# steineggerlab/unicore

Hardware: AMD Instinct MI355X
Metric: 3Di alignments/sec (cluster path) (higher is better)
Workload: dtype u16

## Files before the change

### unicore_amd/csrc/uc_prefilter.hip

```cpp
#include <hip/hip_runtime.h>

#include <algorithm>
#include <cstdlib>
#include <cstring>
#include <type_traits>

#include <rocprim/rocprim.hpp>

#include "uc_engine.h"

namespace uc {

constexpr uint32_t KMER_INVALID = 0xFFFFFFFFu;

struct KmerCfg {
    int koff[K];
    int span;
    int thr;
};

__device__ __forceinline__ uint32_t find_seq(const uint32_t *off, uint32_t lo, uint32_t hi, uint32_t p) {
    while (hi - lo > 1) {
        const uint32_t mid = lo + ((hi - lo) >> 1);
        if (off[mid] <= p) lo = mid; else hi = mid;
// ... 502 lines not shown
            if (base + k < key_cap) keys[base + k] = key;
        }
        __syncthreads();
    }
}

constexpr int FB_LOG2 = 19;
constexpr int FT = 1024;
constexpr int KPT = 4;
constexpr int FILTER_RPT = 2;
constexpr size_t filter_lds(int rpt) { return 2 * ((size_t)1 << FB_LOG2) / 8 + ((size_t)rpt * FT + 1) * 4 + (size_t)rpt * FT * 8 + 16 * 4 + 64; }

__global__ void __launch_bounds__(256) run_range_kernel(const DeviceDb db, uint32_t qbegin, uint32_t nq, uint32_t p0, const uint32_t *rpidx,
                                                        uint64_t n_runs, uint64_t *qr) {
    for (uint32_t i = blockIdx.x * 256 + threadIdx.x; i <= nq; i += gridDim.x * 256) {
        const uint32_t want = db.off[qbegin + i] - p0;
        uint64_t lo = 0, hi = n_runs;
        while (lo < hi) { const uint64_t m = (lo + hi) >> 1; if (rpidx[m] < want) lo = m + 1; else hi = m; }
        qr[i] = lo;
    }
}

__global__ void __launch_bounds__(256) run_order_key_kernel(uint32_t nq, const uint64_t *qr, uint32_t *key, uint32_t *idx) {
    for (uint32_t i = blockIdx.x * 256 + threadIdx.x; i < nq; i += gridDim.x * 256) {
        const uint64_t c = qr[i + 1] - qr[i];
        key[i] = 0xFFFFFFFFu - (uint32_t)min<uint64_t>(c, 0xFFFFFFFFull);
        idx[i] = i;
    }
}

template <bool C> struct TdType { using type = uint64_t; };
template <> struct TdType<true> { using type = uint32_t; };

template <bool C>
__global__ void __launch_bounds__(FT) filter_kernel(const DeviceDb db, uint32_t qbegin, uint32_t p0, const uint32_t *rpidx,
                                                    const uint64_t *rval, const uint64_t *qr, const uint32_t *order, const void *ent, KeyFmt fmt,
                                                    unsigned long long *region_cursor, void *region_v, uint64_t region_cap,
                                                    uint64_t *qbase, uint32_t *qsurv) {
    using TD = typename TdType<C>::type;
    struct __attribute__((aligned(4))) TD4 { TD v[KPT]; };
    TD *region = (TD *)region_v;
    extern __shared__ __attribute__((aligned(16))) uint32_t f_lds[];
    constexpr int BW = 1 << (FB_LOG2 - 5);
    constexpr int RPT = FILTER_RPT;
    constexpr int TR = RPT * FT;
    uint32_t *B1 = f_lds, *B2 = f_lds + BW;
    uint2 *s_run = (uint2 *)(f_lds + 2 * BW);
    uint32_t *s_pref = (uint32_t *)(s_run + TR);
    uint32_t *s_wsum = s_pref + TR + 1;
    uint64_t *s_misc = (uint64_t *)(((uintptr_t)(s_wsum + 16) + 7) & ~(uintptr_t)7);
    const int tid = threadIdx.x, lane = tid & 63, wv = tid >> 6;
    const uint32_t qi = order[blockIdx.x];
    const uint32_t q = qbegin + qi;
    const uint32_t plo = db.off[q] - p0;
    const uint64_t r0 = qr[qi], r1 = qr[qi + 1];
    TD *surv = region + region_cap;
    for (int w = tid; w < 2 * BW; w += FT) f_lds[w] = 0;
    if (r0 == r1) {
        if (tid == 0) { qbase[qi] = 0; qsurv[qi] = 0; }
        return;
    }

    uint64_t pf_rv[RPT] = {};
    uint32_t pf_pi[RPT] = {};
    auto prefetch_tile = [&](uint64_t tile) {
#pragma unroll
        for (int j = 0; j < RPT; j++) {
            const uint64_t r = tile + (uint64_t)RPT * tid + j;
            if (r < r1) { pf_rv[j] = rval[r]; pf_pi[j] = rpidx[r]; }
        }
    };
    auto load_tile = [&](uint64_t tile) {
        uint32_t c[RPT], csum = 0;
#pragma unroll
        for (int j = 0; j < RPT; j++) {
            const uint64_t r = tile + (uint64_t)RPT * tid + j;
            c[j] = r < r1 ? (uint32_t)(pf_rv[j] >> 32) : 0u;
            csum += c[j];
        }
        uint32_t inc = csum;
        for (int o = 1; o < 64; o <<= 1) {
            const uint32_t up = (uint32_t)__shfl_up((int)inc, o, 64);
            if (lane >= o) inc += up;
        }
        if (lane == 63) s_wsum[wv] = inc;
        __syncthreads();
        uint32_t woff = 0;
        for (int w = 0; w < wv; w++) woff += s_wsum[w];
        uint32_t pre = woff + inc - csum;
#pragma unroll
        for (int j = 0; j < RPT; j++) {
            s_pref[RPT * tid + j] = pre;
// ... 160 lines not shown
    __syncthreads();
    auto slot2_of = [&](uint64_t key, uint32_t &h2) -> uint32_t {
        const uint32_t x = (uint32_t)key * 0xC2B2AE35u ^ (uint32_t)(key >> 32) * 0x27D4EB2Fu;
        h2 = ((x ^ (x >> 13)) * 0x165667B1u) >> (32 - FB_LOG2);
        return (x * 0x9E3779B1u) >> (32 - FB_LOG2);
    };
    for (uint32_t k = tid; k < n1; k += FT) {
        uint32_t g;
        const uint32_t h = slot2_of(surv[base + k], g), bit = 1u << (h & 31), gbit = 1u << (g & 31);
        const uint32_t old = atomicOr(&B1[h >> 5], bit);
        if (old & bit) atomicOr(&B2[h >> 5], bit);
        const uint32_t gold = atomicOr(&B1[g >> 5], gbit);
        if (gold & gbit) atomicOr(&B2[g >> 5], gbit);
    }
    __syncthreads();
    const uint32_t n1r = (n1 + 63) / 64 * 64;
    for (uint32_t k = tid; k < n1r; k += FT) {
        TD key = 0;
        bool keep = false;
        if (k < n1) {
            key = surv[base + k];
            uint32_t g;
            const uint32_t h = slot2_of(key, g);
            keep = ((B2[h >> 5] >> (h & 31)) & (B2[g >> 5] >> (g & 31))) & 1u;
        }
        const uint64_t m = __builtin_amdgcn_ballot_w64(keep);
        if (m) {
            uint32_t s0 = 0;
            if (lane == 0) s0 = atomicAdd(cur2, (uint32_t)__popcll(m));
            s0 = (uint32_t)__shfl((int)s0, 0, 64);
            if (keep) region[base + s0 + (uint32_t)__popcll(m & ((1ull << lane) - 1ull))] = key;
        }
    }
    __syncthreads();
    if (tid == 0) { qbase[qi] = base; qsurv[qi] = *cur2; }
}

template <bool C>
__global__ void __launch_bounds__(256) compact_kernel(const void *region_v, const uint64_t *qbase, const uint32_t *qsurv,
                                                      const uint64_t *soff, uint32_t nq, KeyFmt fmt, uint64_t *out) {
    using TD = typename TdType<C>::type;
    const TD *region = (const TD *)region_v;
    const uint64_t dmask = (1ull << fmt.dbits) - 1;
    for (uint32_t b = blockIdx.x; b < nq; b += gridDim.x) {
        const uint64_t src = qbase[b], dst = soff[b];
        const uint32_t n = qsurv[b];
        const uint64_t qbits = (uint64_t)b << (fmt.tbits + fmt.dbits);
        for (uint32_t k = threadIdx.x; k < n; k += 256) {
            const uint64_t td = region[src + k];
            out[dst + k] = C ? (qbits | (((td >> fmt.dbits) + fmt.tbase) << fmt.dbits) | (td & dmask)) : (qbits | td);
        }
    }
}

__global__ void __launch_bounds__(256) diag_select_kernel(const uint64_t *keys, uint64_t n, int min_hits, KeyFmt fmt, uint32_t qbegin,
                                                          unsigned long long *n_cand, uint64_t cap,
                                                          uint32_t *cq, uint32_t *ct, int32_t *cd, uint32_t mirror_q0, uint8_t *wflag) {
    constexpr int DS_SLOTS = 128, DS_DRAIN = 64;
    __shared__ uint32_t s_q[4][DS_SLOTS], s_t[4][DS_SLOTS];
    __shared__ int32_t s_d[4][DS_SLOTS];
    const int lane = threadIdx.x & 63, wv = threadIdx.x >> 6;
    const uint64_t dmask = (1ull << fmt.dbits) - 1, tmask = (1ull << fmt.tbits) - 1;
    const uint64_t nround = (n + 255) / 256 * 256;
    uint32_t staged = 0;
    auto drain = [&]() {
        uint32_t blo = 0, bhi = 0;
        if (lane == 0) {
            const unsigned long long b = atomicAdd(n_cand, (unsigned long long)staged);
// ... 11 lines not shown
    };
    __shared__ uint64_t s_v1[4][64], s_v2[4][64];
    for (uint64_t i = (uint64_t)blockIdx.x * 256 + threadIdx.x; i < nround; i += (uint64_t)gridDim.x * 256) {
        bool cand = false, deferred = false;
        int best_d = 0, last_d = 0;
        uint64_t grp = 0;
        const uint64_t wbase = i - (uint64_t)lane;
        const bool valid = i < n;
        const uint64_t k = valid ? keys[i] : ~0ull;
        uint64_t kp = (uint64_t)__shfl_up((unsigned long long)k, 1, 64);
        if (lane == 0) kp = (valid && i > 0) ? keys[i - 1] : ~k;
        const bool run_start = valid && kp != k;
        const bool grp_start = valid && (i == 0 || (kp >> fmt.dbits) != (k >> fmt.dbits));
        const uint64_t starts = __builtin_amdgcn_ballot_w64(run_start), gstarts = __builtin_amdgcn_ballot_w64(grp_start);
        const uint64_t above = lane == 63 ? 0ull : (~0ull << (lane + 1));
        const uint64_t wend = wbase + 64 < n ? wbase + 64 : n;
        if (grp_start && !(gstarts & above) && wend < n) {
            const uint64_t far = wend + 63 < n ? wend + 63 : n - 1;
            deferred = (keys[far] >> fmt.dbits) == (k >> fmt.dbits);
        }
        const bool long_tail = __builtin_amdgcn_ballot_w64(deferred) != 0;
        uint64_t v1 = 0, v2 = 0;
        if (run_start) {
            const uint64_t nx = starts & above;
            uint64_t cnt;
            if (nx) cnt = (uint64_t)(__builtin_ctzll(nx) - lane);
            else {
                uint64_t e = wend;
                const uint64_t lim = wend + 64 < n ? wend + 64 : n;
                if (!long_tail) while (e < lim && keys[e] == k) e++;
                cnt = e - i;
            }
            const uint64_t d = k & dmask;
            v1 = (cnt << 32) | (0xFFFFFFFFull - d);
            v2 = (cnt << 32) | d;
        }
        s_v1[wv][lane] = v1; s_v2[wv][lane] = v2;
        __builtin_amdgcn_wave_barrier();
        if (grp_start) {
            grp = k >> fmt.dbits;
            const uint64_t ng = gstarts & above;
            const int gend = ng ? __builtin_ctzll(ng) : 64;
            uint64_t b1 = 0, b2 = 0;
            uint64_t runs = starts & (~0ull << lane) & (gend == 64 ? ~0ull : ((1ull << gend) - 1ull));
            while (runs) {
                const int r = __builtin_ctzll(runs);
                runs &= runs - 1;
                const uint64_t a = s_v1[wv][r], c2 = s_v2[wv][r];
                b1 = a > b1 ? a : b1; b2 = c2 > b2 ? c2 : b2;
            }
            if (gend == 64 && wend < n && !deferred) {
                uint64_t e = wend;
                const uint64_t kw = keys[wend - 1];
                while (e < n && keys[e] == kw) e++;
                while (e < n && (keys[e] >> fmt.dbits) == grp) {
                    const uint64_t kb = keys[e];
                    uint64_t f = e + 1;
                    while (f < n && keys[f] == kb) f++;
                    const uint64_t cnt = f - e, d = kb & dmask;
                    const uint64_t a = (cnt << 32) | (0xFFFFFFFFull - d), c2 = (cnt << 32) | d;
                    b1 = a > b1 ? a : b1; b2 = c2 > b2 ? c2 : b2;
                    e = f;
                }
            }
            cand = !deferred && (int)(b1 >> 32) >= min_hits;
            best_d = (int)(0xFFFFFFFFull - (b1 & 0xFFFFFFFFull)) - fmt.dbias;
            last_d = (int)(b2 & 0xFFFFFFFFull) - fmt.dbias;
        }
        __builtin_amdgcn_wave_barrier();
        {
            const uint64_t dm = __builtin_amdgcn_ballot_w64(deferred);
            if (lane == 0 && wbase < n) wflag[wbase >> 6] = dm ? (uint8_t)(__builtin_ctzll(dm) + 1) : (uint8_t)0;
        }
        const uint32_t gq = qbegin + (uint32_t)(grp >> fmt.tbits), gt = (uint32_t)(grp & tmask);
        const uint64_t m = __builtin_amdgcn_ballot_w64(cand);
        if (m) {
            if (cand) {
                const uint32_t k = staged + (uint32_t)__popcll(m & ((1ull << lane) - 1ull));
                s_q[wv][k] = gq;
                s_t[wv][k] = gt;
                s_d[wv][k] = best_d;
            }
            staged += (uint32_t)__popcll(m);
            __builtin_amdgcn_wave_barrier();
            if (staged >= DS_DRAIN) drain();
        }
        const bool mcand = cand && gq >= mirror_q0;
        const uint64_t mm = __builtin_amdgcn_ballot_w64(mcand);
        if (mm) {
            if (mcand) {
                const uint32_t k = staged + (uint32_t)__popcll(mm & ((1ull << lane) - 1ull));
                s_q[wv][k] = gt;
                s_t[wv][k] = gq;
                s_d[wv][k] = -last_d;
            }
            staged += (uint32_t)__popcll(mm);
            __builtin_amdgcn_wave_barrier();
            if (staged >= DS_DRAIN) drain();
        }
    }
// ... 27 lines not shown
    };
    auto wmax = [&](uint64_t v) -> uint64_t {
        for (int o = 32; o > 0; o >>= 1) { const uint64_t x = (uint64_t)__shfl_xor((unsigned long long)v, o, 64); v = x > v ? x : v; }
        return v;
    };
    const uint64_t nw64 = (nwin + 63) >> 6;
    for (uint64_t wb = (uint64_t)blockIdx.x * 4 + wv; wb < nw64; wb += (uint64_t)gridDim.x * 4) {
        const uint64_t w = wb * 64 + lane;
        const uint32_t fl = w < nwin ? wflag[w] : 0u;
        uint64_t pending = __builtin_amdgcn_ballot_w64(fl != 0);
        while (pending) {
            const int src = __builtin_ctzll(pending);
            pending &= pending - 1;
            const uint32_t f = (uint32_t)__shfl((int)fl, src, 64);
            const uint64_t i0 = ((wb * 64 + (uint64_t)src) << 6) + (f - 1);
            const uint64_t grp = keys[i0] >> fmt.dbits;
            uint64_t b1 = 0, b2 = 0, carry_key = 0, carry_cnt = 0;
            bool carry = false;
            for (uint64_t pos = i0;; pos += 64) {
                const uint64_t idx = pos + lane;
                const uint64_t k = idx < n ? keys[idx] : ~0ull;
                const bool in = idx < n && (k >> fmt.dbits) == grp;
                const uint64_t inmask = __builtin_amdgcn_ballot_w64(in);
                const int nin = inmask == ~0ull ? 64 : __builtin_ctzll(~inmask);
                if (nin == 0) break;
                uint64_t kp = (uint64_t)__shfl_up((unsigned long long)k, 1, 64);
                if (lane == 0) kp = carry ? carry_key : ~k;
                const bool rs = lane < nin && kp != k;
                const uint64_t starts = __builtin_amdgcn_ballot_w64(rs);
                const int lead = starts ? __builtin_ctzll(starts) : nin;
                if (carry) {
                    carry_cnt += (uint64_t)lead;
                    if (lead < nin || nin < 64) {
                        const uint64_t d = carry_key & dmask, a = (carry_cnt << 32) | (0xFFFFFFFFull - d), c2 = (carry_cnt << 32) | d;
                        b1 = a > b1 ? a : b1; b2 = c2 > b2 ? c2 : b2;
                        carry = false;
                    }
                }
                const uint64_t above = lane == 63 ? 0ull : (~0ull << (lane + 1));
                uint64_t v1 = 0, v2 = 0;
                bool open = false;
                if (rs) {
                    const uint64_t nx = starts & above;
                    const int end = nx ? __builtin_ctzll(nx) : nin;
                    const uint64_t cnt = (uint64_t)(end - lane), d = k & dmask;
                    open = !nx && nin == 64;
                    if (!open) { v1 = (cnt << 32) | (0xFFFFFFFFull - d); v2 = (cnt << 32) | d; }
                }
                v1 = wmax(v1); v2 = wmax(v2);
                b1 = v1 > b1 ? v1 : b1; b2 = v2 > b2 ? v2 : b2;
                const uint64_t om = __builtin_amdgcn_ballot_w64(open);
                if (om) {
                    const int ol = __builtin_ctzll(om);
                    carry_key = (uint64_t)__shfl((unsigned long long)k, ol, 64);
                    carry_cnt = (uint64_t)(64 - ol);
                    carry = true;
                }
                if (nin < 64) break;
            }
            if (carry) {
                const uint64_t d = carry_key & dmask, a = (carry_cnt << 32) | (0xFFFFFFFFull - d), c2 = (carry_cnt << 32) | d;
                b1 = a > b1 ? a : b1; b2 = c2 > b2 ? c2 : b2;
            }
            if ((int)(b1 >> 32) >= min_hits) {
                const uint32_t gq = qbegin + (uint32_t)(grp >> fmt.tbits), gt = (uint32_t)(grp & tmask);
                const bool mir = gq >= mirror_q0;
                if (lane == 0) {
                    s_q[wv][staged] = gq; s_t[wv][staged] = gt; s_d[wv][staged] = (int)(0xFFFFFFFFull - (b1 & 0xFFFFFFFFull)) - fmt.dbias;
                    if (mir) { s_q[wv][staged + 1] = gt; s_t[wv][staged + 1] = gq; s_d[wv][staged + 1] = -((int)(b2 & 0xFFFFFFFFull) - fmt.dbias); }
                }
                staged += mir ? 2u : 1u;
                __builtin_amdgcn_wave_barrier();
                if (staged >= 64) drain();
            }
        }
    }
    if (staged) drain();
}

__global__ void __launch_bounds__(256) select_key_kernel(uint64_t n, const uint32_t *cq, const uint32_t *ct, const int32_t *score,
                                                         int min_score, uint64_t *key, unsigned long long *n_kept) {
    unsigned long long kept = 0;
    for (uint64_t i = (uint64_t)blockIdx.x * 256 + threadIdx.x; i < n; i += (uint64_t)gridDim.x * 256) {
        const int s = score[i];
        const bool ok = s >= min_score;
        key[i] = ok ? ((uint64_t)cq[i] << 32) | ((uint64_t)(255 - s) << 24) | ct[i] : ~0ull;
        kept += ok;
    }
    for (int o = 32; o > 0; o >>= 1) kept += __shfl_down(kept, o, 64);
    if ((threadIdx.x & 63) == 0 && kept) atomicAdd(n_kept, kept);
}

__global__ void __launch_bounds__(256) rank_flag_kernel(const uint64_t *skey, uint64_t n, uint32_t max_seqs, uint32_t *flag) {
    for (uint64_t i = (uint64_t)blockIdx.x * 256 + threadIdx.x; i < n; i += (uint64_t)gridDim.x * 256) {
        const uint64_t qk = skey[i] & 0xFFFFFFFF00000000ull;
        flag[i] = (i < max_seqs || skey[i - max_seqs] < qk) ? 1u : 0u;
    }
}

__global__ void __launch_bounds__(256) hit_scatter_kernel(const uint64_t *skey, const int32_t *sdiag, uint64_t n, const uint32_t *flag,
                                                          const uint64_t *pos, uint32_t *hq, uint32_t *ht, int32_t *hs, int32_t *hd) {
    for (uint64_t i = (uint64_t)blockIdx.x * 256 + threadIdx.x; i < n; i += (uint64_t)gridDim.x * 256) {
// ... 36 lines not shown
    for (uint64_t i = (uint64_t)blockIdx.x * 256 + threadIdx.x; i < n; i += (uint64_t)gridDim.x * 256)
        if (flag[i] && pair_owner((uint32_t)(skey[i] >> 32), (uint32_t)(skey[i] & 0xFFFFFFu), len, world) != rank) flag[i] = 0;
}

__global__ void __launch_bounds__(256) owner_key_kernel(uint64_t n, const uint32_t *hq, const uint32_t *ht, const uint32_t *len, uint32_t world,
                                                        uint32_t *okey, uint32_t *idx, unsigned long long *count ) {
    for (uint64_t i = (uint64_t)blockIdx.x * 256 + threadIdx.x; i < n; i += (uint64_t)gridDim.x * 256) {
        const uint32_t o = pair_owner(hq[i], ht[i], len, world);
        okey[i] = o;
        idx[i] = (uint32_t)i;
        for (uint32_t w = 0; w < world; w++) {
            const unsigned long long m = __ballot(o == w);
            if (m && (threadIdx.x & 63) == (unsigned)__ffsll((long long)m) - 1) atomicAdd(count + w, (unsigned long long)__popcll(m));
        }
    }
}
__global__ void __launch_bounds__(256) owner_gather_kernel(uint64_t n, const uint32_t *idx, const uint32_t *hq, const uint32_t *ht, const int32_t *hs,
                                                           const int32_t *hd, uint32_t *oq, uint32_t *ot, int32_t *os, int32_t *od) {
    for (uint64_t i = (uint64_t)blockIdx.x * 256 + threadIdx.x; i < n; i += (uint64_t)gridDim.x * 256) {
        const uint32_t j = idx[i];
        oq[i] = hq[j]; ot[i] = ht[j]; os[i] = hs[j]; od[i] = hd[j];
    }
}

struct WidenU32 {
    __host__ __device__ uint64_t operator()(uint32_t x) const { return (uint64_t)x; }
};

struct PrefilterScratch {
    DevBuf<unsigned long long> d_counters;
    DevBuf<char> d_temp;
    DevBuf<uint32_t> d_koff, k_in, k_out, d_ent32, v_in32, d_okey, d_okey2, d_oidx, d_order;
    DevBuf<uint64_t> d_ent, v_in;
    DevBuf<uint32_t> d_cnt, d_flag, d_cq, d_ct, d_rpidx2, d_qsurv;
    DevBuf<uint64_t> d_keys, d_keys2, d_pos, d_skey, d_skey2, d_rval2, d_qbase, d_soff, d_qr;
    DevBuf<int32_t> d_cd, d_cd2, d_score, d_mval;
    DevBuf<uint64_t> d_mkey;
    DevBuf<uint32_t> acc_q, acc_t, pass_q, pass_t;
    DevBuf<int32_t> acc_s, acc_d, pass_s, pass_d;
    DevBuf<uint8_t> d_kflag, d_wflag;
    DevBuf<uint32_t> d_qk, d_kid, d_dk, d_nsimk, d_drk, d_drk2, d_roff, d_nr, d_src, d_ph;
    DevBuf<uint64_t> d_drv, d_drv2, d_cumh, d_cumr, d_qh, d_qrn;
    DevBuf<RankRec> d_rec;
    DevBuf<uint32_t> d_kbits;
    UngappedAllWork ua;
    template <class F> void each(F f) {
        f(d_counters); f(d_temp); f(d_koff); f(k_in); f(k_out); f(d_ent32); f(v_in32); f(d_okey); f(d_okey2); f(d_oidx); f(d_order);
        f(d_ent); f(v_in); f(d_cnt); f(d_flag); f(d_cq); f(d_ct); f(d_rpidx2); f(d_qsurv); f(d_keys); f(d_keys2); f(d_pos); f(d_skey);
        f(d_skey2); f(d_rval2); f(d_qbase); f(d_soff); f(d_qr); f(d_cd); f(d_cd2); f(d_score); f(d_kflag); f(d_wflag); f(d_qk); f(d_kid); f(d_dk);
        f(d_nsimk); f(d_drk); f(d_drk2); f(d_roff); f(d_nr); f(d_src); f(d_ph); f(d_drv); f(d_drv2); f(d_cumh); f(d_cumr); f(d_qh); f(d_qrn); f(d_rec); f(d_kbits); f(d_mkey); f(d_mval); f(acc_q); f(acc_t); f(pass_q); f(pass_t); f(acc_s); f(acc_d); f(pass_s); f(pass_d);
        f(ua.score); f(ua.diag); f(ua.pairs); f(ua.prof); f(ua.prof_off);
    }
    size_t bytes() {
        size_t b = 0;
        each([&](auto &x) { b += x.cap * sizeof(*x.p); });
        return b;
    }
    void release_bytes(size_t target) {
        if (getenv("UC_TIMING")) {
            fprintf(stderr, "unicore-cluster[timing]: prefilter scratch %.1f GiB, %.1f GiB to give back before the gapped stage; buffers >= 2 GiB (index in PrefilterScratch::each: GiB):", bytes() / 1073741824.0, target / 1073741824.0);
            int i = 0;
            each([&](auto &x) { const double g = x.cap * sizeof(*x.p) / 1073741824.0; if (g >= 2.0) fprintf(stderr, " %d:%.1f", i, g); i++; });
            fprintf(stderr, "\n");
        }
        if (!target) return;
        if (target >= bytes()) { each([&](auto &x) { if (x.cap * sizeof(*x.p) >= ((size_t)1 << 30)) x.release(); }); return; }
        size_t freed = 0;
        while (freed < target) {
            size_t best = 0;
            each([&](auto &x) { best = std::max(best, x.cap * sizeof(*x.p)); });
            if (best < ((size_t)256 << 20)) break;
            bool done = false;
            each([&](auto &x) { if (!done && x.cap * sizeof(*x.p) == best) { x.release(); done = true; } });
            freed += best;
        }
    }
};
void free_scratch(PrefilterScratch *p) { delete p; }

static size_t scratch_release_target(bool gapped_stage_sizes_by_free_memory, uint64_t n_hits, size_t scratch_bytes, bool gapped_scratch_warm) {
    size_t fr = 0, tot = 0;
    if (hipMemGetInfo(&fr, &tot) != hipSuccess || tot == 0) return scratch_bytes > ((size_t)96 << 30) ? scratch_bytes : 0;
// ... 28 lines not shown
    for (uint32_t q = 0; q < n; q++) hit_off[q + 1] = hit_off[q] + hit_cnt[q];
    if (hit_off[n] != n_hits) fail(UC_ERR_GENERIC, "%s: hit list bookkeeping mismatch", who);
}

constexpr uint64_t RUN_MAX = 1ull << 29;
struct PrefilterPass {
    KmerCfg cfg;
    KeyFmt fmt;
    uint32_t tbegin = 0, tend = 0;
    uint32_t qbegin = 0, qend = 0;
    uint32_t mirror_q0 = UINT32_MAX;
    bool count_sims = false;
    double density_limit = 0.0, *density_out = nullptr;
    const void *ent_p = nullptr;
    uint32_t n_entries = 0;
    uint64_t HIT_CAP = 0, HIT_CAP_BIG = 0, DRUN_MAX = 0;
    uint64_t n_hits_total = 0, n_cand_total = 0, cand_cap = 0, run_cap = 1ull << 20;
    double t_kmer = 0, t_ung = 0, t_sel = 0, gpu_ms = 0;
};
struct SuperBatch {
    uint32_t begin = 0, end = 0;
    uint32_t P0 = 0, NP = 0;
    std::vector<uint64_t> h_qh, h_qr;
    uint64_t hit_cap = 0;
    double frac = 1.0;
};
struct QueryBatch {
    uint32_t qa = 0, qb = 0;
    uint64_t total_hits = 0, n_runs = 0;
    uint32_t qp0 = 0, qp1 = 0, nq_res = 0;
    unsigned kbits = 0;
    const uint64_t *sorted = nullptr;
    uint64_t n_sort = 0;
};
static KeyFmt key_format(const Engine &E, uint32_t tbegin, uint32_t tend) {
    KeyFmt fmt;
    const uint32_t m = std::min<uint32_t>(std::max<uint32_t>(E.max_len, 2), 65536u);
    fmt.dbits = 1;
    while ((1u << (fmt.dbits - 1)) < m) fmt.dbits++;
    fmt.dbias = 1 << (fmt.dbits - 1);
    fmt.tbits = 1;
    while ((1u << fmt.tbits) < E.hdb.n) fmt.tbits++;
    int rbits = 1;
    while ((1ull << rbits) < (uint64_t)std::max<uint32_t>(tend - tbegin, 1)) rbits++;
    fmt.compact = rbits + fmt.dbits <= 32 && !getenv("UC_PREFILTER_WIDE");
    fmt.tbase = tbegin;
    return fmt;
}

static void build_index(Engine &E, PrefilterPass &PP) {
    PrefilterScratch &S = *E.pre;
    Timer t_index;
    E.timed_ms_begin();
    const uint32_t tp0 = E.h_poff[PP.tbegin], tp1 = E.h_poff[PP.tend];
    const uint32_t nres = tp1 - tp0;
    S.d_koff.reserve((size_t)KSPACE + 1);
    PP.fmt = key_format(E, PP.tbegin, PP.tend);
    const KeyFmt &fmt = PP.fmt;
    const size_t cap = std::max<uint32_t>(nres, 1);
    S.k_in.reserve(cap); S.k_out.reserve(cap);
    if (fmt.compact) { S.v_in32.reserve(cap); S.d_ent32.reserve(cap); PP.ent_p = S.d_ent32.p; }
    else { S.v_in.reserve(cap); S.d_ent.reserve(cap); PP.ent_p = S.d_ent.p; }
    if (nres) {
        hipLaunchKernelGGL(kmer_extract_kernel, grid_for(nres), dim3(256), 0, E.stream, E.ddb, PP.tbegin, PP.tend, PP.cfg, tp0, tp1, S.k_in.p,
                           fmt.compact ? nullptr : S.v_in.p, fmt.compact ? S.v_in32.p : nullptr, fmt.dbits - 1);
        if (fmt.compact)
// ... 150 lines not shown
        const uint64_t h = SB.h_qh[B.qb - SB.begin], r = SB.h_qr[B.qb - SB.begin];
        if (B.qb > qa && (B.total_hits + h > SB.hit_cap || B.n_runs + r > RUN_MAX)) break;
        B.total_hits += h; B.n_runs += r;
        if (B.qb >= PP.mirror_q0) mirror_hits += h;
        B.qb++;
    }
    if (B.n_runs >= (1ull << 32)) fail(UC_ERR_GENERIC, "query %u alone produces %llu index ranges", qa, (unsigned long long)B.n_runs);
    B.qp0 = E.h_poff[qa]; B.qp1 = E.h_poff[B.qb]; B.nq_res = B.qp1 - B.qp0;
    PP.run_cap = std::max<uint64_t>(PP.run_cap, B.n_runs);
    S.d_rpidx2.reserve(PP.run_cap); S.d_rval2.reserve(PP.run_cap);
    UC_HIP(hipMemsetAsync(S.d_counters.p + 3, 0, 32, E.stream));
    if (B.n_runs)
        hipLaunchKernelGGL(position_expand_kernel, grid_for(B.nq_res), dim3(256), 0, E.stream, B.qp0 - SB.P0, B.qp1 - SB.P0, S.d_nr.p, S.d_src.p, S.d_cumr.p, S.d_drv2.p,
                           S.d_rpidx2.p, S.d_rval2.p);
    if (B.total_hits > (1ull << 34)) fail(UC_ERR_GENERIC, "query %u alone produces %llu k-mer hits", qa, (unsigned long long)B.total_hits);
    PP.n_hits_total += B.total_hits + mirror_hits;
    unsigned qbits = 1;
    while ((1u << qbits) < B.qb - qa) qbits++;
    B.kbits = (unsigned)(PP.fmt.dbits + PP.fmt.tbits) + qbits;
    return B;
}

static uint64_t compact_u64(Engine &E, DevBuf<char> &tmp, uint32_t *cnt, uint64_t *pos, uint64_t n, const uint32_t *also = nullptr, uint32_t *also_out = nullptr) {
    auto in = rocprim::make_transform_iterator(cnt, WidenU32());
    rocprim_call(tmp, [&](void *t, size_t &b) { return rocprim::exclusive_scan(t, b, in, pos, (uint64_t)0, (size_t)n, rocprim::plus<uint64_t>(), E.stream); });
    uint64_t lp = 0; uint32_t lc = 0;
    UC_HIP(hipMemcpyAsync(&lp, pos + (n - 1), 8, hipMemcpyDeviceToHost, E.stream));
    UC_HIP(hipMemcpyAsync(&lc, cnt + (n - 1), 4, hipMemcpyDeviceToHost, E.stream));
    if (also) UC_HIP(hipMemcpyAsync(also_out, also, 4, hipMemcpyDeviceToHost, E.stream));
    UC_HIP(hipStreamSynchronize(E.stream));
    return lp + lc;
}

static void expand_keys_filtered(Engine &E, PrefilterPass &PP, QueryBatch &B) {
    PrefilterScratch &S = *E.pre;
    const KeyFmt &fmt = PP.fmt;
    const uint32_t qa = B.qa, qp0 = B.qp0, nq = B.qb - B.qa;
    S.d_qbase.reserve(nq); S.d_qsurv.reserve(nq); S.d_soff.reserve((size_t)nq + 1);
    const uint64_t region_cap = B.total_hits + (uint64_t)KPT * nq;
    S.d_keys.reserve(fmt.compact ? region_cap : 2 * region_cap);
    S.d_qr.reserve((size_t)nq + 1);
    hipLaunchKernelGGL(run_range_kernel, grid_for((uint64_t)nq + 1), dim3(256), 0, E.stream, E.ddb, qa, nq, qp0, S.d_rpidx2.p, B.n_runs, S.d_qr.p);
    S.d_okey.reserve(nq); S.d_okey2.reserve(nq); S.d_oidx.reserve(nq); S.d_order.reserve(nq);
    hipLaunchKernelGGL(run_order_key_kernel, grid_for(nq), dim3(256), 0, E.stream, nq, S.d_qr.p, S.d_okey.p, S.d_oidx.p);
    rocprim_call(S.d_temp, [&](void *t, size_t &b) { return rocprim::radix_sort_pairs(t, b, S.d_okey.p, S.d_okey2.p, S.d_oidx.p, S.d_order.p, (size_t)nq, 0u, 32u, E.stream); });
    auto launch = [&](auto kern) {
        static PerDeviceOnce once[2];
        once[fmt.compact ? 1 : 0]([&] { UC_HIP(hipFuncSetAttribute((const void *)kern, hipFuncAttributeMaxDynamicSharedMemorySize, (int)filter_lds(FILTER_RPT))); });
        hipLaunchKernelGGL(kern, dim3(nq), dim3(FT), filter_lds(FILTER_RPT), E.stream, E.ddb, qa, qp0, S.d_rpidx2.p, S.d_rval2.p, S.d_qr.p, S.d_order.p, PP.ent_p, fmt,
                           S.d_counters.p + 5, (void *)S.d_keys.p, region_cap, S.d_qbase.p, S.d_qsurv.p);
    };
    if (fmt.compact) launch(filter_kernel<true>);
    else launch(filter_kernel<false>);
    const uint64_t n_sort = compact_u64(E, S.d_temp, S.d_qsurv.p, S.d_soff.p, nq);
    if (n_sort) {
        S.d_keys2.reserve(2 * n_sort);
        hipLaunchKernelGGL(fmt.compact ? compact_kernel<true> : compact_kernel<false>, dim3(std::min<uint32_t>(nq, 65535u)), dim3(256), 0, E.stream,
                           (const void *)S.d_keys.p, S.d_qbase.p, S.d_qsurv.p, S.d_soff.p, nq, fmt, S.d_keys2.p);
        rocprim_call(S.d_temp, [&](void *t, size_t &b) { return rocprim::radix_sort_keys(t, b, S.d_keys2.p, S.d_keys2.p + n_sort, (size_t)n_sort, 0u, B.kbits, E.stream); });
    }
    B.sorted = S.d_keys2.p + n_sort; B.n_sort = n_sort;
    E.stats.n_filtered_hits += n_sort;
}

static void expand_keys_plain(Engine &E, PrefilterPass &PP, QueryBatch &B) {
    PrefilterScratch &S = *E.pre;
    S.d_keys.reserve(B.total_hits); S.d_keys2.reserve(B.total_hits);
    const RunList rl{S.d_rpidx2.p, S.d_rval2.p, PP.run_cap};
    hipLaunchKernelGGL(expand_kernel, grid_for(B.n_runs), dim3(256), 0, E.stream, E.ddb, B.qa, B.qb, B.qp0, rl, B.n_runs, PP.ent_p, PP.fmt,
                       S.d_counters.p + 5, S.d_keys.p, B.total_hits);
    rocprim_call(S.d_temp, [&](void *t, size_t &b) { return rocprim::radix_sort_keys(t, b, S.d_keys.p, S.d_keys2.p, (size_t)B.total_hits, 0u, B.kbits, E.stream); });
    B.sorted = S.d_keys2.p; B.n_sort = B.total_hits;
    E.stats.n_filtered_hits += B.n_sort;
}

static uint64_t select_diagonals(Engine &E, PrefilterPass &PP, const QueryBatch &B) {
    PrefilterScratch &S = *E.pre;
    PP.cand_cap = std::max<uint64_t>(PP.cand_cap, std::max<uint64_t>(1u << 20, B.total_hits / 32));
    for (;;) {
        S.d_cq.reserve(PP.cand_cap); S.d_ct.reserve(PP.cand_cap); S.d_cd.reserve(PP.cand_cap);
        UC_HIP(hipMemsetAsync(S.d_counters.p + 6, 0, 8, E.stream));
        if (B.n_sort) {
            S.d_wflag.reserve((B.n_sort + 63) / 64 + 64);
            hipLaunchKernelGGL(diag_select_kernel, grid_for(B.n_sort), dim3(256), 0, E.stream, B.sorted, B.n_sort, E.p.min_diag_hits, PP.fmt, B.qa,
                               S.d_counters.p + 6, PP.cand_cap, S.d_cq.p, S.d_ct.p, S.d_cd.p, PP.mirror_q0, S.d_wflag.p);
            hipLaunchKernelGGL(diag_long_kernel, grid_for((B.n_sort + 63) / 64), dim3(256), 0, E.stream, B.sorted, B.n_sort, E.p.min_diag_hits, PP.fmt, B.qa,
                               S.d_counters.p + 6, PP.cand_cap, S.d_cq.p, S.d_ct.p, S.d_cd.p, PP.mirror_q0, (const uint8_t *)S.d_wflag.p);
        }
        unsigned long long nc = 0;
        UC_HIP(hipMemcpyAsync(&nc, S.d_counters.p + 6, 8, hipMemcpyDeviceToHost, E.stream));
        UC_HIP(hipStreamSynchronize(E.stream));
        if (nc <= PP.cand_cap) return nc;
        PP.cand_cap = nc;
    }
}

static void rescore_ungapped(Engine &E, PrefilterPass &PP, uint64_t n_cand) {
    PrefilterScratch &S = *E.pre;
    Timer t_u;
    E.timed_ms_begin();
    S.d_score.reserve(n_cand);
    launch_ungapped(E.ddb, n_cand, S.d_cq.p, S.d_ct.p, S.d_cd.p, S.d_score.p, S.d_counters.p + 2, E.stream);
    UC_HIP(hipGetLastError());
    PP.gpu_ms += E.timed_ms_end();
    PP.t_ung += t_u.seconds();
}

static void select_and_append(Engine &E, PrefilterPass &PP, uint64_t n_cand) {
    PrefilterScratch &S = *E.pre;
    Timer t_s;
    E.timed_ms_begin();
    S.d_skey.reserve(n_cand); S.d_skey2.reserve(n_cand); S.d_cd2.reserve(n_cand);
    UC_HIP(hipMemsetAsync(S.d_counters.p + 1, 0, 8, E.stream));
    hipLaunchKernelGGL(select_key_kernel, grid_for(n_cand), dim3(256), 0, E.stream, n_cand, S.d_cq.p, S.d_ct.p, S.d_score.p, E.p.min_ungapped, S.d_skey.p, S.d_counters.p + 1);
    rocprim_call(S.d_temp, [&](void *t, size_t &b) { return rocprim::radix_sort_pairs(t, b, S.d_skey.p, S.d_skey2.p, S.d_cd.p, S.d_cd2.p, (size_t)n_cand, 0u, 64u, E.stream); });
    unsigned long long kept = 0;
    UC_HIP(hipMemcpyAsync(&kept, S.d_counters.p + 1, 8, hipMemcpyDeviceToHost, E.stream));
    UC_HIP(hipStreamSynchronize(E.stream));
    if (kept) {
        S.d_flag.reserve(kept); S.d_pos.reserve(kept);
        hipLaunchKernelGGL(rank_flag_kernel, grid_for(kept), dim3(256), 0, E.stream, S.d_skey2.p, (uint64_t)kept, (uint32_t)E.p.max_seqs, S.d_flag.p);
        const uint64_t add = compact_u64(E, S.d_temp, S.d_flag.p, S.d_pos.p, kept), n_hits = E.n_hits;
        E.d_hq.grow_preserve(n_hits + add, n_hits, E.stream); E.d_ht.grow_preserve(n_hits + add, n_hits, E.stream);
        E.d_hs.grow_preserve(n_hits + add, n_hits, E.stream); E.d_hd.grow_preserve(n_hits + add, n_hits, E.stream);
        hipLaunchKernelGGL(hit_scatter_kernel, grid_for(kept), dim3(256), 0, E.stream, S.d_skey2.p, S.d_cd2.p, (uint64_t)kept, S.d_flag.p, S.d_pos.p,
                           E.d_hq.p + n_hits, E.d_ht.p + n_hits, E.d_hs.p + n_hits, E.d_hd.p + n_hits);
// ... 347 lines not shown
```

Measured before the change: 22.43 million.

## Select diagonals on-chip in filter kernel for small per-query survivor sets

When a query's filtered survivor count fits in LDS, the filter kernel now bitonic-sorts the keys in shared memory, computes per-diagonal run counts and best/last diagonal per target, and writes candidates directly. A new gather kernel scatters these into the candidate arrays, and only the overflow queries still go through the compact, global radix-sort and diag_select path. This avoids the global sort and extra kernel passes for most queries, but adds per-block sorting work, extra scans and host copies, and a new code path that could diverge from the global selection semantics.

```diff
diff --git a/unicore_amd/csrc/uc_prefilter.hip b/unicore_amd/csrc/uc_prefilter.hip
--- a/unicore_amd/csrc/uc_prefilter.hip
+++ b/unicore_amd/csrc/uc_prefilter.hip
@@ -558,11 +558,22 @@
 template <bool C> struct TdType { using type = uint64_t; };
 template <> struct TdType<true> { using type = uint32_t; };
 
+template <class R> __device__ __forceinline__ R diag_rank_fwd(R cnt, R d, int sh) { return (cnt << sh) | (((((R)1 << sh) - 1)) - d); }
+template <class R> __device__ __forceinline__ R diag_rank_rev(R cnt, R d, int sh) { return (cnt << sh) | d; }
+template <class R> __device__ __forceinline__ bool diag_pick(R b1, R b2, int sh, int min_hits, int dbias, int &best_d, int &last_d) {
+    const R m = ((R)1 << sh) - 1;
+    best_d = (int)(m - (b1 & m)) - dbias;
+    last_d = (int)(b2 & m) - dbias;
+    return (int)(b1 >> sh) >= min_hits;
+}
+constexpr uint32_t TAIL_MAX = 12288;
+
 template <bool C>
 __global__ void __launch_bounds__(FT) filter_kernel(const DeviceDb db, uint32_t qbegin, uint32_t p0, const uint32_t *rpidx,
                                                     const uint64_t *rval, const uint64_t *qr, const uint32_t *order, const void *ent, KeyFmt fmt,
                                                     unsigned long long *region_cursor, void *region_v, uint64_t region_cap,
-                                                    uint64_t *qbase, uint32_t *qsurv) {
+                                                    uint64_t *qbase, uint32_t *qsurv, uint32_t tail_limit, int min_hits, uint32_t mirror_q0,
+                                                    uint32_t *qcand, unsigned long long *n_tail_keys) {
     using TD = typename TdType<C>::type;
     struct __attribute__((aligned(4))) TD4 { TD v[KPT]; };
     TD *region = (TD *)region_v;
@@ -583,7 +594,7 @@
     TD *surv = region + region_cap;
     for (int w = tid; w < 2 * BW; w += FT) f_lds[w] = 0;
     if (r0 == r1) {
-        if (tid == 0) { qbase[qi] = 0; qsurv[qi] = 0; }
+        if (tid == 0) { qbase[qi] = 0; qsurv[qi] = 0; qcand[qi] = 0; }
         return;
     }
 
@@ -810,8 +821,106 @@
             if (keep) region[base + s0 + (uint32_t)__popcll(m & ((1ull << lane) - 1ull))] = key;
         }
     }
+    __threadfence_block();
     __syncthreads();
-    if (tid == 0) { qbase[qi] = base; qsurv[qi] = *cur2; }
+    const uint32_t n2 = *cur2;
+    if (!C || tail_limit == 0 || n2 > tail_limit) {
+        if (tid == 0) { qbase[qi] = base; qsurv[qi] = n2; qcand[qi] = 0; }
+        return;
+    }
+    if constexpr (C) {
+        static_assert(3 * TAIL_MAX <= 2 * BW + 2 * TR + TR && TAIL_MAX < (1u << 14), "tail arrays fit the dead LDS; a run count fits 14 bits");
+        uint32_t *sk = f_lds, *a1 = f_lds + TAIL_MAX, *a2 = f_lds + 2 * TAIL_MAX;
+        for (uint32_t k = tid; k < n2; k += FT) { sk[k] = region[base + k]; a1[k] = 0; a2[k] = 0; }
+        __syncthreads();
+        int lnp = 0;
+        while ((1u << lnp) < n2) lnp++;
+        const uint32_t half = lnp ? 1u << (lnp - 1) : 0u;
+        auto cmpx = [&](uint32_t i, uint32_t l) {
+            if (l < n2) {
+                const uint32_t a = sk[i], b = sk[l];
+                if (a > b) { sk[i] = b; sk[l] = a; }
+            }
+        };
+        for (int lk = 1; lk <= lnp; lk++) {
+            for (uint32_t c = tid; c < half; c += FT) {
+                const uint32_t b0 = (c >> (lk - 1)) << lk, o = c & ((1u << (lk - 1)) - 1u);
+                cmpx(b0 + o, b0 + ((1u << lk) - 1u - o));
+            }
+            __syncthreads();
+            for (int lj = lk - 2; lj >= 0; lj--) {
+                for (uint32_t c = tid; c < half; c += FT) {
+                    const uint32_t i = ((c >> lj) << (lj + 1)) + (c & ((1u << lj) - 1u));
+                    cmpx(i, i + (1u << lj));
+                }
+                __syncthreads();
+            }
+        }
+        const uint32_t dm = (1u << fmt.dbits) - 1u;
+        for (uint32_t i = tid; i < n2; i += FT) {
+            const uint32_t k = sk[i];
+            if (i && sk[i - 1] == k) continue;
+            uint32_t lo = i + 1, hi = n2;
+            while (lo < hi) { const uint32_t m = (lo + hi) >> 1; if (sk[m] <= k) lo = m + 1; else hi = m; }
+            const uint32_t cnt = lo - i, g = k & ~dm;
+            uint32_t glo = 0, ghi = i;
+            while (glo < ghi) { const uint32_t m = (glo + ghi) >> 1; if (sk[m] < g) glo = m + 1; else ghi = m; }
+            atomicMax(&a1[glo], diag_rank_fwd<uint32_t>(cnt, k & dm, fmt.dbits));
+            atomicMax(&a2[glo], diag_rank_rev<uint32_t>(cnt, k & dm, fmt.dbits));
+        }
+        __syncthreads();
+        const uint32_t slab = (n2 + FT - 1) / FT * 64;
+        const uint32_t s0 = min(n2, (uint32_t)wv * slab), s1 = min(n2, s0 + slab);
+        auto group_at = [&](uint32_t i, uint32_t &gt, int &bd, int &ld) -> uint32_t {
+            if (i >= s1) return 0u;
+            const uint32_t k = sk[i];
+            if (i && (sk[i - 1] >> fmt.dbits) == (k >> fmt.dbits)) return 0u;
+            if (!diag_pick<uint32_t>(a1[i], a2[i], fmt.dbits, min_hits, fmt.dbias, bd, ld)) return 0u;
+            gt = (k >> fmt.dbits) + fmt.tbase;
+            return q >= mirror_q0 ? 2u : 1u;
+        };
+        uint32_t mine = 0;
+        for (uint32_t i0 = s0; i0 < s1; i0 += 64) {
+            uint32_t gt; int bd, ld;
+            mine += group_at(i0 + lane, gt, bd, ld);
+        }
+        for (int o = 32; o > 0; o >>= 1) mine += (uint32_t)__shfl_down((int)mine, o, 64);
+        if (lane == 0) s_wsum[wv] = mine;
+        __syncthreads();
+        uint32_t off = 0, tot = 0;
+        for (int w = 0; w < FT / 64; w++) { if (w < wv) off += s_wsum[w]; tot += s_wsum[w]; }
+        const uint64_t below = (1ull << lane) - 1ull;
+        for (uint32_t i0 = s0; i0 < s1; i0 += 64) {
+            uint32_t gt = 0; int bd = 0, ld = 0;
+            const uint32_t nrec = group_at(i0 + lane, gt, bd, ld);
+            const uint64_t m1 = __builtin_amdgcn_ballot_w64(nrec >= 1), m2 = __builtin_amdgcn_ballot_w64(nrec == 2);
+            const uint32_t pos = off + (uint32_t)__popcll(m1 & below) + (uint32_t)__popcll(m2 & below);
+            if (nrec && pos + nrec <= n2) {
+                region[base + pos] = gt; surv[base + pos] = (uint32_t)bd;
+                if (nrec == 2) { region[base + pos + 1] = gt | 0x80000000u; surv[base + pos + 1] = (uint32_t)(-ld); }
+            }
+            off += (uint32_t)__popcll(m1) + (uint32_t)__popcll(m2);
+        }
+        if (tid == 0) {
+            qbase[qi] = base; qsurv[qi] = 0; qcand[qi] = tot;
+            atomicAdd(n_tail_keys, (unsigned long long)n2);
+        }
+    }
+}
+
+__global__ void __launch_bounds__(256) tail_gather_kernel(const uint32_t *region, uint64_t region_cap, const uint64_t *qbase, const uint32_t *qcand,
+                                                          const uint64_t *coff, uint32_t nq, uint32_t qbegin, uint32_t *cq, uint32_t *ct, int32_t *cd) {
+    for (uint32_t b = blockIdx.x; b < nq; b += gridDim.x) {
+        const uint64_t src = qbase[b], dst = coff[b];
+        const uint32_t n = qcand[b], q = qbegin + b;
+        for (uint32_t k = threadIdx.x; k < n; k += 256) {
+            const uint32_t a = region[src + k], t = a & 0x7FFFFFFFu;
+            const bool rev = a >> 31;
+            cq[dst + k] = rev ? t : q;
+            ct[dst + k] = rev ? q : t;
+            cd[dst + k] = (int32_t)region[region_cap + src + k];
+        }
+    }
 }
 
 template <bool C>
@@ -889,8 +998,8 @@
                 cnt = e - i;
             }
             const uint64_t d = k & dmask;
-            v1 = (cnt << 32) | (0xFFFFFFFFull - d);
-            v2 = (cnt << 32) | d;
+            v1 = diag_rank_fwd<uint64_t>(cnt, d, 32);
+            v2 = diag_rank_rev<uint64_t>(cnt, d, 32);
         }
         s_v1[wv][lane] = v1; s_v2[wv][lane] = v2;
         __builtin_amdgcn_wave_barrier();
@@ -915,14 +1024,12 @@
                     uint64_t f = e + 1;
                     while (f < n && keys[f] == kb) f++;
                     const uint64_t cnt = f - e, d = kb & dmask;
-                    const uint64_t a = (cnt << 32) | (0xFFFFFFFFull - d), c2 = (cnt << 32) | d;
+                    const uint64_t a = diag_rank_fwd<uint64_t>(cnt, d, 32), c2 = diag_rank_rev<uint64_t>(cnt, d, 32);
                     b1 = a > b1 ? a : b1; b2 = c2 > b2 ? c2 : b2;
                     e = f;
                 }
             }
-            cand = !deferred && (int)(b1 >> 32) >= min_hits;
-            best_d = (int)(0xFFFFFFFFull - (b1 & 0xFFFFFFFFull)) - fmt.dbias;
-            last_d = (int)(b2 & 0xFFFFFFFFull) - fmt.dbias;
+            cand = diag_pick<uint64_t>(b1, b2, 32, min_hits, fmt.dbias, best_d, last_d) && !deferred;
         }
         __builtin_amdgcn_wave_barrier();
         {
@@ -1016,7 +1123,7 @@
                 if (carry) {
                     carry_cnt += (uint64_t)lead;
                     if (lead < nin || nin < 64) {
-                        const uint64_t d = carry_key & dmask, a = (carry_cnt << 32) | (0xFFFFFFFFull - d), c2 = (carry_cnt << 32) | d;
+                        const uint64_t d = carry_key & dmask, a = diag_rank_fwd<uint64_t>(carry_cnt, d, 32), c2 = diag_rank_rev<uint64_t>(carry_cnt, d, 32);
                         b1 = a > b1 ? a : b1; b2 = c2 > b2 ? c2 : b2;
                         carry = false;
                     }
@@ -1029,7 +1136,7 @@
                     const int end = nx ? __builtin_ctzll(nx) : nin;
                     const uint64_t cnt = (uint64_t)(end - lane), d = k & dmask;
                     open = !nx && nin == 64;
-                    if (!open) { v1 = (cnt << 32) | (0xFFFFFFFFull - d); v2 = (cnt << 32) | d; }
+                    if (!open) { v1 = diag_rank_fwd<uint64_t>(cnt, d, 32); v2 = diag_rank_rev<uint64_t>(cnt, d, 32); }
                 }
                 v1 = wmax(v1); v2 = wmax(v2);
                 b1 = v1 > b1 ? v1 : b1; b2 = v2 > b2 ? v2 : b2;
@@ -1043,15 +1150,16 @@
                 if (nin < 64) break;
             }
             if (carry) {
-                const uint64_t d = carry_key & dmask, a = (carry_cnt << 32) | (0xFFFFFFFFull - d), c2 = (carry_cnt << 32) | d;
+                const uint64_t d = carry_key & dmask, a = diag_rank_fwd<uint64_t>(carry_cnt, d, 32), c2 = diag_rank_rev<uint64_t>(carry_cnt, d, 32);
                 b1 = a > b1 ? a : b1; b2 = c2 > b2 ? c2 : b2;
             }
-            if ((int)(b1 >> 32) >= min_hits) {
+            int best_d, last_d;
+            if (diag_pick<uint64_t>(b1, b2, 32, min_hits, fmt.dbias, best_d, last_d)) {
                 const uint32_t gq = qbegin + (uint32_t)(grp >> fmt.tbits), gt = (uint32_t)(grp & tmask);
                 const bool mir = gq >= mirror_q0;
                 if (lane == 0) {
-                    s_q[wv][staged] = gq; s_t[wv][staged] = gt; s_d[wv][staged] = (int)(0xFFFFFFFFull - (b1 & 0xFFFFFFFFull)) - fmt.dbias;
-                    if (mir) { s_q[wv][staged + 1] = gt; s_t[wv][staged + 1] = gq; s_d[wv][staged + 1] = -((int)(b2 & 0xFFFFFFFFull) - fmt.dbias); }
+                    s_q[wv][staged] = gq; s_t[wv][staged] = gt; s_d[wv][staged] = best_d;
+                    if (mir) { s_q[wv][staged + 1] = gt; s_t[wv][staged + 1] = gq; s_d[wv][staged + 1] = -last_d; }
                 }
                 staged += mir ? 2u : 1u;
                 __builtin_amdgcn_wave_barrier();
@@ -1154,8 +1262,8 @@
     DevBuf<char> d_temp;
     DevBuf<uint32_t> d_koff, k_in, k_out, d_ent32, v_in32, d_okey, d_okey2, d_oidx, d_order;
     DevBuf<uint64_t> d_ent, v_in;
-    DevBuf<uint32_t> d_cnt, d_flag, d_cq, d_ct, d_rpidx2, d_qsurv;
-    DevBuf<uint64_t> d_keys, d_keys2, d_pos, d_skey, d_skey2, d_rval2, d_qbase, d_soff, d_qr;
+    DevBuf<uint32_t> d_cnt, d_flag, d_cq, d_ct, d_rpidx2, d_qsurv, d_qcand;
+    DevBuf<uint64_t> d_keys, d_keys2, d_pos, d_skey, d_skey2, d_rval2, d_qbase, d_soff, d_coff, d_qr;
     DevBuf<int32_t> d_cd, d_cd2, d_score, d_mval;
     DevBuf<uint64_t> d_mkey;
     DevBuf<uint32_t> acc_q, acc_t, pass_q, pass_t;
@@ -1169,7 +1277,7 @@
     template <class F> void each(F f) {
         f(d_counters); f(d_temp); f(d_koff); f(k_in); f(k_out); f(d_ent32); f(v_in32); f(d_okey); f(d_okey2); f(d_oidx); f(d_order);
         f(d_ent); f(v_in); f(d_cnt); f(d_flag); f(d_cq); f(d_ct); f(d_rpidx2); f(d_qsurv); f(d_keys); f(d_keys2); f(d_pos); f(d_skey);
-        f(d_skey2); f(d_rval2); f(d_qbase); f(d_soff); f(d_qr); f(d_cd); f(d_cd2); f(d_score); f(d_kflag); f(d_wflag); f(d_qk); f(d_kid); f(d_dk);
+        f(d_skey2); f(d_rval2); f(d_qbase); f(d_soff); f(d_qr); f(d_cd); f(d_cd2); f(d_score); f(d_qcand); f(d_coff); f(d_kflag); f(d_wflag); f(d_qk); f(d_kid); f(d_dk);
         f(d_nsimk); f(d_drk); f(d_drk2); f(d_roff); f(d_nr); f(d_src); f(d_ph); f(d_drv); f(d_drv2); f(d_cumh); f(d_cumr); f(d_qh); f(d_qrn); f(d_rec); f(d_kbits); f(d_mkey); f(d_mval); f(acc_q); f(acc_t); f(pass_q); f(pass_t); f(acc_s); f(acc_d); f(pass_s); f(pass_d);
         f(ua.score); f(ua.diag); f(ua.pairs); f(ua.prof); f(ua.prof_off);
     }
@@ -1264,6 +1372,7 @@
     unsigned kbits = 0;
     const uint64_t *sorted = nullptr;
     uint64_t n_sort = 0;
+    uint64_t n_tail_cand = 0, region_cap = 0;
 };
 static KeyFmt key_format(const Engine &E, uint32_t tbegin, uint32_t tend) {
     KeyFmt fmt;
@@ -1480,11 +1589,17 @@
     return lp + lc;
 }
 
+static uint32_t onchip_tail_limit(const Engine &E, const KeyFmt &fmt) {
+    const char *on = getenv("UC_PREFILTER_ONCHIP"), *lim = getenv("UC_PREFILTER_ONCHIP_LIMIT");
+    if (!fmt.compact || fmt.dbits + 14 > 32 || E.p.min_diag_hits < 2 || (on && atoi(on) == 0)) return 0;
+    return lim ? (uint32_t)std::min<unsigned long long>(TAIL_MAX, strtoull(lim, nullptr, 10)) : TAIL_MAX;
+}
+
 static void expand_keys_filtered(Engine &E, PrefilterPass &PP, QueryBatch &B) {
     PrefilterScratch &S = *E.pre;
     const KeyFmt &fmt = PP.fmt;
     const uint32_t qa = B.qa, qp0 = B.qp0, nq = B.qb - B.qa;
-    S.d_qbase.reserve(nq); S.d_qsurv.reserve(nq); S.d_soff.reserve((size_t)nq + 1);
+    S.d_qbase.reserve(nq); S.d_qsurv.reserve(nq); S.d_soff.reserve((size_t)nq + 1); S.d_qcand.reserve(nq); S.d_coff.reserve((size_t)nq + 1);
     const uint64_t region_cap = B.total_hits + (uint64_t)KPT * nq;
     S.d_keys.reserve(fmt.compact ? region_cap : 2 * region_cap);
     S.d_qr.reserve((size_t)nq + 1);
@@ -1496,11 +1611,20 @@
         static PerDeviceOnce once[2];
         once[fmt.compact ? 1 : 0]([&] { UC_HIP(hipFuncSetAttribute((const void *)kern, hipFuncAttributeMaxDynamicSharedMemorySize, (int)filter_lds(FILTER_RPT))); });
         hipLaunchKernelGGL(kern, dim3(nq), dim3(FT), filter_lds(FILTER_RPT), E.stream, E.ddb, qa, qp0, S.d_rpidx2.p, S.d_rval2.p, S.d_qr.p, S.d_order.p, PP.ent_p, fmt,
-                           S.d_counters.p + 5, (void *)S.d_keys.p, region_cap, S.d_qbase.p, S.d_qsurv.p);
+                           S.d_counters.p + 5, (void *)S.d_keys.p, region_cap, S.d_qbase.p, S.d_qsurv.p, onchip_tail_limit(E, fmt), E.p.min_diag_hits, PP.mirror_q0,
+                           S.d_qcand.p, S.d_counters.p + 7);
     };
+    UC_HIP(hipMemsetAsync(S.d_counters.p + 7, 0, 8, E.stream));
     if (fmt.compact) launch(filter_kernel<true>);
     else launch(filter_kernel<false>);
+    auto cin = rocprim::make_transform_iterator(S.d_qcand.p, WidenU32());
+    rocprim_call(S.d_temp, [&](void *t, size_t &b) { return rocprim::exclusive_scan(t, b, cin, S.d_coff.p, (uint64_t)0, (size_t)nq, rocprim::plus<uint64_t>(), E.stream); });
+    uint64_t cp = 0; uint32_t cc = 0; unsigned long long n_tail_keys = 0;
+    UC_HIP(hipMemcpyAsync(&cp, S.d_coff.p + (nq - 1), 8, hipMemcpyDeviceToHost, E.stream));
+    UC_HIP(hipMemcpyAsync(&cc, S.d_qcand.p + (nq - 1), 4, hipMemcpyDeviceToHost, E.stream));
+    UC_HIP(hipMemcpyAsync(&n_tail_keys, S.d_counters.p + 7, 8, hipMemcpyDeviceToHost, E.stream));
     const uint64_t n_sort = compact_u64(E, S.d_temp, S.d_qsurv.p, S.d_soff.p, nq);
+    B.n_tail_cand = cp + cc; B.region_cap = region_cap;
     if (n_sort) {
         S.d_keys2.reserve(2 * n_sort);
         hipLaunchKernelGGL(fmt.compact ? compact_kernel<true> : compact_kernel<false>, dim3(std::min<uint32_t>(nq, 65535u)), dim3(256), 0, E.stream,
@@ -1508,7 +1632,7 @@
         rocprim_call(S.d_temp, [&](void *t, size_t &b) { return rocprim::radix_sort_keys(t, b, S.d_keys2.p, S.d_keys2.p + n_sort, (size_t)n_sort, 0u, B.kbits, E.stream); });
     }
     B.sorted = S.d_keys2.p + n_sort; B.n_sort = n_sort;
-    E.stats.n_filtered_hits += n_sort;
+    E.stats.n_filtered_hits += n_sort + n_tail_keys;
 }
 
 static void expand_keys_plain(Engine &E, PrefilterPass &PP, QueryBatch &B) {
@@ -1524,22 +1648,29 @@
 
 static uint64_t select_diagonals(Engine &E, PrefilterPass &PP, const QueryBatch &B) {
     PrefilterScratch &S = *E.pre;
-    PP.cand_cap = std::max<uint64_t>(PP.cand_cap, std::max<uint64_t>(1u << 20, B.total_hits / 32));
+    const uint64_t nt = B.n_tail_cand;
+    PP.cand_cap = std::max<uint64_t>(PP.cand_cap, nt + std::max<uint64_t>(1u << 20, B.total_hits / 32));
     for (;;) {
         S.d_cq.reserve(PP.cand_cap); S.d_ct.reserve(PP.cand_cap); S.d_cd.reserve(PP.cand_cap);
+        if (nt)
+            hipLaunchKernelGGL(tail_gather_kernel, dim3(std::min<uint32_t>(B.qb - B.qa, 65535u)), dim3(256), 0, E.stream, (const uint32_t *)S.d_keys.p, B.region_cap,
+                               S.d_qbase.p, S.d_qcand.p, S.d_coff.p, B.qb - B.qa, B.qa, S.d_cq.p, S.d_ct.p, S.d_cd.p);
+        if (!B.n_sort) {
+            UC_HIP(hipStreamSynchronize(E.stream));
+            return nt;
+        }
+        const uint64_t cap = PP.cand_cap - nt;
         UC_HIP(hipMemsetAsync(S.d_counters.p + 6, 0, 8, E.stream));
-        if (B.n_sort) {
-            S.d_wflag.reserve((B.n_sort + 63) / 64 + 64);
-            hipLaunchKernelGGL(diag_select_kernel, grid_for(B.n_sort), dim3(256), 0, E.stream, B.sorted, B.n_sort, E.p.min_diag_hits, PP.fmt, B.qa,
-                               S.d_counters.p + 6, PP.cand_cap, S.d_cq.p, S.d_ct.p, S.d_cd.p, PP.mirror_q0, S.d_wflag.p);
-            hipLaunchKernelGGL(diag_long_kernel, grid_for((B.n_sort + 63) / 64), dim3(256), 0, E.stream, B.sorted, B.n_sort, E.p.min_diag_hits, PP.fmt, B.qa,
-                               S.d_counters.p + 6, PP.cand_cap, S.d_cq.p, S.d_ct.p, S.d_cd.p, PP.mirror_q0, (const uint8_t *)S.d_wflag.p);
-        }
+        S.d_wflag.reserve((B.n_sort + 63) / 64 + 64);
+        hipLaunchKernelGGL(diag_select_kernel, grid_for(B.n_sort), dim3(256), 0, E.stream, B.sorted, B.n_sort, E.p.min_diag_hits, PP.fmt, B.qa,
+                           S.d_counters.p + 6, cap, S.d_cq.p + nt, S.d_ct.p + nt, S.d_cd.p + nt, PP.mirror_q0, S.d_wflag.p);
+        hipLaunchKernelGGL(diag_long_kernel, grid_for((B.n_sort + 63) / 64), dim3(256), 0, E.stream, B.sorted, B.n_sort, E.p.min_diag_hits, PP.fmt, B.qa,
+                           S.d_counters.p + 6, cap, S.d_cq.p + nt, S.d_ct.p + nt, S.d_cd.p + nt, PP.mirror_q0, (const uint8_t *)S.d_wflag.p);
         unsigned long long nc = 0;
         UC_HIP(hipMemcpyAsync(&nc, S.d_counters.p + 6, 8, hipMemcpyDeviceToHost, E.stream));
         UC_HIP(hipStreamSynchronize(E.stream));
-        if (nc <= PP.cand_cap) return nc;
-        PP.cand_cap = nc;
+        if (nc <= cap) return nt + nc;
+        PP.cand_cap = nt + nc;
     }
 }
 
```

Result: no change. 22.41 million, median of 2 (-0.1%).
